# QWERTY6191/projected-lmc

Measured on AMD Instinct MI355X. Metric: MLL+grad iters/sec, n=8192 16-task LMC, higher is better.
Workload: dtype f32; 1 GPU; C3: ProjectedGPModel+ProjectedLMCmll exact training step (PLMC_fast), n=8192 d=8 p=16 q=8 Matern-5/2 fp32; latents sharded q/N per GPU; n_points=8192, n_dim=8, n_tasks=16, n_latents=8, parallelism=latent-shard x1

## Files before the change

projected-lmc_amd/csrc/api_common.hpp:

```cpp
#pragma once
#include <hip/hip_runtime.h>
#include <stdint.h>
#include <stdio.h>
#include <string.h>
#include <type_traits>

#include "gemm_core.hpp"
#include "covariance.hpp"

namespace plmc {

constexpr int MAX_DIM = 32;
constexpr int MAX_COMP = 4;
constexpr int SM_MAX_MIX = 8;
constexpr int SM_MAX_DIM = 8;
constexpr int PER_MAX_DIM = 8;
constexpr int RQ_MAX_DIM = 16;
constexpr int LPER_MAX_DIM = 8;
constexpr int DOT_MAX_DIM = 16;
constexpr int DOT_MAX_POWER = 8;
constexpr int SUM_MAX_DIM = 8;
constexpr int FAM_PUBLIC_BASE = 16;
enum { F_PER = 5, F_RQ = 6, F_LPER = 7 };

// ... 112 lines not shown
  static CovTable add(int kind, int d, int ncomp, const void *ell, const void *oscale) { return {COV_ADD, kind, d, ncomp, ell, nullptr, oscale}; }
  static CovTable sm(int d, int nmix, const void *scales, const void *means, const void *weights) { return {COV_SM, 0, d, nmix, scales, means, weights}; }
  static CovTable per(int d, const void *ell, const void *period, const void *oscale) { return {COV_PER, 0, d, 1, ell, period, oscale}; }
  static CovTable rq(int d, const void *ell, const void *alpha, const void *oscale) { return {COV_RQ, 0, d, 1, ell, alpha, oscale}; }
  static CovTable lper(int d, const void *ell, const void *period, const void *rbf_ell, const void *oscale) {
    return {COV_LPER, 0, d, 1, ell, period, oscale, rbf_ell};
  }
  static CovTable dot(int d, int power, const void *v, const void *c, const void *oscale) { return {COV_DOT, 0, d, power, v, c, oscale}; }
  int power() const { return ncomp; }
  static CovTable sum(int d, int ncomp, const int *fam, const void *table, const void *oscale) {
    CovTable t{COV_SUM, 0, d, ncomp, table, nullptr, oscale};
    if (!fam) t.fams = -3;
    if (!fam || ncomp < 1 || ncomp > MAX_COMP) return t;
    for (int g = 0; g < ncomp; ++g) {
      const int f = fam[g];
      int code;
      if (f >= K_RBF && f <= K_MATERN52) code = f;
      else if (f >= FAM_PUBLIC_BASE && f <= FAM_PUBLIC_BASE + 2) code = F_PER + (f - FAM_PUBLIC_BASE);
      else { t.fams = f == K_SPLINE ? -2 : -1; return t; }
      t.fams |= code << (4 * g);
    }
    return t;
  }
  int fam_of(int g) const { return (fams >> (4 * g)) & 15; }
  CovTable member(const void *ell_, const void *period_, const void *rbf_, const void *alpha_, const void *os_) const {
    const int f = fam_of(0);
    CovTable t = f == F_PER ? per(d, ell_, period_, os_) : f == F_RQ ? rq(d, ell_, alpha_, os_) : f == F_LPER ? lper(d, ell_, period_, rbf_, os_)
                                                                                                          : plain(f, d, ell_, os_);
    t.of_sum = true;
    return t;
  }
  template <typename T> CovTable member_of_latent(int lat) const {
    const T *rec = (const T *)ell + (int64_t)lat * (3 * d + 1);
    return member(rec, rec + d, rec + 2 * d, rec + 3 * d, oscale ? (const T *)oscale + lat : nullptr);
  }
  bool single_member() const { return family == COV_SUM && ncomp == 1; }
  const char *check() const {
    const FamilyTraits &f = FAMILY[family];
    if (family == COV_ADD && (kind < 0 || kind > K_MATERN52)) return "additive kernels take the stationary kinds only (no spline kernel)";
    const char *count = f.max_count && (ncomp < 1 || ncomp > f.max_count) ? f.count_text : nullptr;
    const char *dim = f.max_dim && (d <= 0 || d > f.max_dim) ? f.dim_text : nullptr;
    if (count || dim) return f.count_first ? (count ? count : dim) : (dim ? dim : count);
    if (family == COV_SUM) {
      if (fams == -3 || !ell) return "null pointer";
      if (fams == -2) return "the spline kernel is not a member of a sum (members: the stationary kinds 0..3, PLMC_FAM_PERIODIC, PLMC_FAM_RQ, PLMC_FAM_LPER)";
      if (fams < 0) return "unknown member family code (members: the stationary kinds 0..3, PLMC_FAM_PERIODIC, PLMC_FAM_RQ, PLMC_FAM_LPER; no spectral mixture)";
    }
    return (f.needs_third && !third) || (f.needs_second && !second) ? "null pointer" : nullptr;
  }
  CovFamily route() const { return family == COV_ADD && ncomp == 1 ? COV_PLAIN : family; }
  int partials_rows() const { return FAMILY[family].rows_per_comp ? ncomp : 1; }
  int kernel_kind() const { return family == COV_SUM ? fams : kind; }
  const char *vd_noun() const { return FAMILY[of_sum ? COV_SUM : route()].vd_noun; }
};
#define PLMC_REQUIRE_TABLE(t) \
  do { if (const char *why_ = (t).check()) return plmc::fail(__func__, why_); } while (0)

#define PLMC_LEAD_KIND int kind,
#define PLMC_LEAD_NO_KIND
#define PLMC_UNPACK(...) __VA_ARGS__
#define PLMC_FAMILY_ENTRIES(X, SUF, T)                                                                                                        \
  X(SUF, T, , KIND, (const T *ell, const T *oscale), plmc::CovTable::plain(kind, d, ell, oscale))                                             \
  X(SUF, T, _add, KIND, (int ncomp, const T *ell, const T *oscale), plmc::CovTable::add(kind, d, ncomp, ell, oscale))                         \
  X(SUF, T, _sm, NO_KIND, (int nmix, const T *scales, const T *means, const T *weights), plmc::CovTable::sm(d, nmix, scales, means, weights)) \
  X(SUF, T, _per, NO_KIND, (const T *ell, const T *period, const T *oscale), plmc::CovTable::per(d, ell, period, oscale))                     \
  X(SUF, T, _rq, NO_KIND, (const T *ell, const T *shape, const T *oscale), plmc::CovTable::rq(d, ell, shape, oscale))                         \
  X(SUF, T, _lper, NO_KIND, (const T *ell, const T *period, const T *rbf_ell, const T *oscale),                                               \
    plmc::CovTable::lper(d, ell, period, rbf_ell, oscale))                                                                                    \
  X(SUF, T, _sum, NO_KIND, (int ncomp, const int *fam, const T *table, const T *oscale), plmc::CovTable::sum(d, ncomp, fam, table, oscale))   \
  X(SUF, T, _dot, NO_KIND, (const T *var, const T *offset, int power, const T *oscale), plmc::CovTable::dot(d, power, var, offset, oscale))

struct AssembleJob {
  CovTable table;
  int n;
  const void *X, *noise;
  const void *pnoise = nullptr;
  int64_t stride_pn = 0;
};
#define PLMC_REQUIRE_POINT_NOISE(pnoise, stride_pn, n)                                                                                        \
  do {                                                                                                                                        \
    PLMC_REQUIRE((pnoise) != nullptr, "null pointer");                                                                                        \
    PLMC_REQUIRE((stride_pn) == 0 || (stride_pn) >= (n), "bad sizes (stride_pn is 0, one vector for every latent, or >= n)");                 \
  } while (0)
int assemble_rows(const AssembleJob &job, int elem_bytes, void *A, int64_t lda, int64_t strideA, int q, int ib0, int nrows, void *stream,
                  int ncols = -1, int skip = 0);

hipStream_t side_stream(int which = 0);
hipEvent_t sync_event(int idx);
void bind_sweep_ctx(hipStream_t caller, int e_prev_idx);

inline bool aligned16(const void *p) { return (reinterpret_cast<uintptr_t>(p) & 15) == 0; }

}
```

projected-lmc_amd/csrc/assemble.hip:

```cpp
#include "api_common.hpp"
#include "covariance.hpp"
#include "cov_tables.hpp"
#include "../../include/plmc.h"

namespace plmc {

#define PLMC_ASSEMBLE_BODY(PN)                                                                                                          \
  const int jb = blockIdx.x, ib = ib0 + blockIdx.y, lat = blockIdx.z;                                                                   \
  if (jb < ib || (ib < skip && jb < skip)) return;    \
  extern __shared__ __align__(16) unsigned char smem_raw[];                                                                             \
  T *ui = reinterpret_cast<T *>(smem_raw);                                                                                              \
  const int ldu = d + 1;                                                                                                                \
  T *uj = ui + NB * ldu;                                                                                                                \
  const int tid = threadIdx.x;                                                                                                          \
  const T *el = ell + (int64_t)lat * d;                                                                                                 \
  for (int e = tid; e < NB * d; e += NTHREADS) {                                                                                        \
    int r = e / d, k = e % d;                                                                                                           \
    int gi = ib * NB + r, gj = jb * NB + r;                                                                                             \
    T inv = T(1) / el[k];                                                                                                               \
    ui[r * ldu + k] = gi < n ? X[(int64_t)gi * d + k] * inv : T(0);                                                                     \
    uj[r * ldu + k] = gj < n ? X[(int64_t)gj * d + k] * inv : T(0);                                                                     \
  }                                                                                                                                     \
  __syncthreads();                                                                                                                      \
  const T os = oscale ? oscale[lat] : T(1);                                                                                             \
  const T nz = noise[lat];                                                                                                              \
  T *Al = A + (int64_t)lat * strideA;                                                                                                   \
  const int tx = tid & 15, ty = tid >> 4;                                                                                               \
  _Pragma("unroll 1")                                                                                                                   \
  for (int rr = 0; rr < 8; ++rr) {                                                                                                      \
    const int r = ty + 16 * rr;                                                                                                         \
    const int gi = ib * NB + r;                                                                                                         \
    T pv = T(0);                                                                                                                        \
    if (PN && ib == jb) pv = pnoise[(int64_t)lat * stride_pn + (gi < n ? gi : n - 1)];    \
  _Pragma("unroll")                                                                                                                     \
    for (int h = 0; h < 2; ++h) {                                                                                                       \
      const int c0 = tx * 4 + 64 * h;                                                                                                   \
      T v[4];                                                                                                                           \
  _Pragma("unroll")                                                                                                                     \
      for (int c = 0; c < 4; ++c) {                                                                                                     \
        const int gj = jb * NB + c0 + c;                                                                                                \
        T r2 = T(0), sp = T(1);                                                                                                         \
        for (int k = 0; k < d; ++k) {                                                                                                   \
          T df = ui[r * ldu + k] - uj[(c0 + c) * ldu + k];                                                                              \
          r2 += df * df;                                                                                                                \
          if (kind == K_SPLINE) sp *= spline_factor(ui[r * ldu + k], uj[(c0 + c) * ldu + k]);                                           \
        }                                                                                                                               \
        T val;                                                                                                                          \
        if (gi < n && gj < n) {                                                                                                         \
          val = os * (kind == K_SPLINE ? sp : kern_value<T>(kind, r2));                                                                 \
          if (gi == gj) { val += nz; if (PN) val += pv; }                                                                               \
        } else {                                                                                                                        \
          val = (gi == gj) ? T(1) : T(0);                                         \
        }                                                                                                                               \
        v[c] = val;                                                                                                                     \
      }                                                                                                                                 \
      T *dst = Al + (int64_t)gi * lda + jb * NB + c0;                                  \
      using vec_t = typename Traits<T>::vec_t;                                                                                          \
      constexpr int EPV = Traits<T>::EPV;                                                                                               \
  _Pragma("unroll")                                                                                                                     \
      for (int c = 0; c < 4; c += EPV) {                                                                                                \
        vec_t o;                                                                                                                        \
  _Pragma("unroll")                                                                                                                     \
        for (int e = 0; e < EPV; ++e) o[e] = v[c + e];                                                                                  \
        *reinterpret_cast<vec_t *>(dst + c) = o;                                                                                        \
      }                                                                                                                                 \
    }                                                                                                                                   \
  }
template <typename T>
__global__ __launch_bounds__(NTHREADS) void k_assemble(int kind, const T *__restrict__ X, int n, int d,
                                                        const T *__restrict__ ell, const T *__restrict__ oscale,
                                                        const T *__restrict__ noise, T *__restrict__ A,
                                                        int64_t lda, int64_t strideA, int ib0, int skip) {
  const T *const pnoise = nullptr;
  const int64_t stride_pn = 0;
  PLMC_ASSEMBLE_BODY(false)
}
template <typename T>
__global__ __launch_bounds__(NTHREADS) void k_assemble_pn(int kind, const T *__restrict__ X, int n, int d,
                                                           const T *__restrict__ ell, const T *__restrict__ oscale,
                                                           const T *__restrict__ noise, const T *__restrict__ pnoise, int64_t stride_pn,
                                                           T *__restrict__ A, int64_t lda, int64_t strideA, int ib0, int skip) {
  PLMC_ASSEMBLE_BODY(true)
}

template <typename T, int DCAP, int KIND, class NZ>
__device__ __forceinline__ void assemble_tile(const T *ui, const T *uj, int ldu, T os, NZ nz, T *Al, int64_t lda, int ib,
                                              int jb, int n, bool edge) {
  typedef Pair<T> T2;
  const int tid = threadIdx.x, tx = tid & 31, ty = tid >> 5;
  const int c0 = tx * 4;
  T2 u2[2][DCAP];
#pragma unroll
  for (int pp = 0; pp < 2; ++pp)
#pragma unroll
    for (int k = 0; k < DCAP; ++k) u2[pp][k] = T2{uj[(c0 + 2 * pp) * ldu + k], uj[(c0 + 2 * pp + 1) * ldu + k]};
#pragma unroll 2
  for (int rr = 0; rr < 16; ++rr) {
    const int r = ty + 8 * rr;
    const int gi = ib * NB + r;
    T xi[DCAP];
#pragma unroll
    for (int k = 0; k < DCAP; ++k) xi[k] = ui[r * ldu + k];
    T2 v[2];
#pragma unroll
    for (int pp = 0; pp < 2; ++pp) {
      T2 r2 = {T(0), T(0)};
#pragma unroll
      for (int k = 0; k < DCAP; ++k) {
        const T2 df = xi[k] - u2[pp][k];
        r2 += df * df;
      }
      v[pp] = os * kern_value_pair<T>(KIND, r2);
    }
    T o[4] = {v[0].x, v[0].y, v[1].x, v[1].y};
    if (edge) {
      const auto rn = row_noise<T>(nz, gi, n, ib == jb);
#pragma unroll
      for (int c = 0; c < 4; ++c) {
        const int gj = jb * NB + c0 + c;
        if (gi < n && gj < n) { if (gi == gj) o[c] = add_noise<T>(o[c], rn); }
        else o[c] = (gi == gj) ? T(1) : T(0);
      }
    }
    T *dst = Al + (int64_t)gi * lda + jb * NB + c0;
    using vec_t = typename Traits<T>::vec_t;
    constexpr int EPV = Traits<T>::EPV;
#pragma unroll
    for (int c = 0; c < 4; c += EPV) {
      vec_t w;
#pragma unroll
      for (int e = 0; e < EPV; ++e) w[e] = o[c + e];
      *reinterpret_cast<vec_t *>(dst + c) = w;
    }
  }
}

#define PLMC_ASSEMBLE_SMALL_BODY(PN)                                                                                \
  const int jb = blockIdx.x, ib = ib0 + blockIdx.y, lat = blockIdx.z;                                               \
  if (jb < ib || (ib < skip && jb < skip)) return;                                                                  \
  constexpr int ldu = DCAP + 1;                                                                                     \
  __shared__ T ui[NB * ldu], uj[NB * ldu];                                                                          \
  const int tid = threadIdx.x;                                                                                      \
  const T *el = ell + (int64_t)lat * d;                                                                             \
  for (int e = tid; e < NB * DCAP; e += NTHREADS) {    \
    const int r = e / DCAP, k = e % DCAP;                                                                           \
    const int gi = ib * NB + r, gj = jb * NB + r;                                                                   \
    const T inv = k < d ? T(1) / el[k] : T(0);                                                                      \
    ui[r * ldu + k] = (k < d && gi < n) ? X[(int64_t)gi * d + k] * inv : T(0);                                      \
    uj[r * ldu + k] = (k < d && gj < n) ? X[(int64_t)gj * d + k] * inv : T(0);                                      \
  }                                                                                                                 \
  __syncthreads();                                                                                                  \
  const T os = oscale ? oscale[lat] : T(1);                                                                         \
  const std::conditional_t<PN, PointNoise<T>, T> nz = diag_noise_of<T, PN>(noise, pnoise, stride_pn, lat);          \
  T *Al = A + (int64_t)lat * strideA;                                                                               \
  const bool edge = ib == jb || (jb + 1) * NB > n;                                                                  \
  if (kind == K_RBF) assemble_tile<T, DCAP, K_RBF>(ui, uj, ldu, os, nz, Al, lda, ib, jb, n, edge);                  \
  else if (kind == K_MATERN12) assemble_tile<T, DCAP, K_MATERN12>(ui, uj, ldu, os, nz, Al, lda, ib, jb, n, edge);   \
  else if (kind == K_MATERN32) assemble_tile<T, DCAP, K_MATERN32>(ui, uj, ldu, os, nz, Al, lda, ib, jb, n, edge);   \
  else assemble_tile<T, DCAP, K_MATERN52>(ui, uj, ldu, os, nz, Al, lda, ib, jb, n, edge);
template <typename T, int DCAP>
__global__ __launch_bounds__(NTHREADS) void k_assemble_small(int kind, const T *__restrict__ X, int n, int d,
                                                              const T *__restrict__ ell, const T *__restrict__ oscale,
                                                              const T *__restrict__ noise, T *__restrict__ A,
                                                              int64_t lda, int64_t strideA, int ib0, int skip) {
  const T *const pnoise = nullptr;
  const int64_t stride_pn = 0;
  PLMC_ASSEMBLE_SMALL_BODY(false)
}
template <typename T, int DCAP>
__global__ __launch_bounds__(NTHREADS) void k_assemble_small_pn(int kind, const T *__restrict__ X, int n, int d,
                                                                 const T *__restrict__ ell, const T *__restrict__ oscale,
                                                                 const T *__restrict__ noise, const T *__restrict__ pnoise,
                                                                 int64_t stride_pn, T *__restrict__ A, int64_t lda, int64_t strideA,
                                                                 int ib0, int skip) {
  PLMC_ASSEMBLE_SMALL_BODY(true)
}

template <typename T>
__global__ void k_write_rhs(const T *__restrict__ rhs, int nrhs, int n, T *__restrict__ A, int64_t n_pad,
                            int64_t lda, int64_t strideA, int c0, int64_t naug_pad, int zero_fill) {
  const int lat = blockIdx.y;
  const int64_t idx = (int64_t)blockIdx.x * blockDim.x + threadIdx.x;
  if (idx >= n_pad * naug_pad) return;
  const int64_t i = idx / naug_pad;
  const int c = (int)(idx % naug_pad);
  T *p = A + (int64_t)lat * strideA + i * lda + n_pad + c;
  if (c >= c0 && c < c0 + nrhs) {
    *p = i < n ? rhs[((int64_t)lat * nrhs + (c - c0)) * n + i] : T(0);
  } else if (zero_fill) {
    *p = T(0);
  }
}

constexpr int CROSS_ROWS = 32;
template <typename T, int DCAP>
__global__ __launch_bounds__(NTHREADS) void k_assemble_cross(int kind, const T *__restrict__ X, int n,
                                                              const T *__restrict__ Xs, int ns, int d,
                                                              const T *__restrict__ ell, const T *__restrict__ oscale,
                                                              T *__restrict__ A, int64_t n_rows, int64_t lda,
                                                              int64_t strideA, int64_t col0) {
  __shared__ T xi[CROSS_ROWS][DCAP + 1];
  const int lat = blockIdx.z;
  const int j = blockIdx.x * NTHREADS + threadIdx.x;
  const int64_t i0 = (int64_t)blockIdx.y * CROSS_ROWS;
  const T *el = ell + (int64_t)lat * d;
  for (int e = threadIdx.x; e < CROSS_ROWS * DCAP; e += NTHREADS) {
    const int r = e / DCAP, k = e % DCAP;
    xi[r][k] = (k < d && i0 + r < n) ? X[(i0 + r) * d + k] / el[k] : T(0);
  }
  T xs[DCAP];
#pragma unroll
  for (int k = 0; k < DCAP; ++k) xs[k] = (k < d && j < ns) ? Xs[(int64_t)j * d + k] / el[k] : T(0);
  const T os = oscale ? oscale[lat] : T(1);
  __syncthreads();
  if (j >= ns) return;
  T *out = A + (int64_t)lat * strideA + i0 * lda + col0 + j;
#pragma unroll 4
  for (int r = 0; r < CROSS_ROWS; ++r) {
    if (i0 + r >= n_rows) break;
    T val = T(0);
    if (i0 + r < n) {
      T r2 = T(0), sp = T(1);
#pragma unroll
      for (int k = 0; k < DCAP; ++k) {
        const T df = xi[r][k] - xs[k];
        r2 += df * df;
        if (kind == K_SPLINE && k < d) sp *= spline_factor(xi[r][k], xs[k]);
      }
      val = os * (kind == K_SPLINE ? sp : kern_value<T>(kind, r2));
    }
    out[(int64_t)r * lda] = val;
  }
}

#define PLMC_ASSEMBLE_SMALL_TABLE_BODY(PN)                                                                          \
  const int jb = blockIdx.x, ib = ib0 + blockIdx.y, lat = blockIdx.z;                                               \
  if (jb < ib || (ib < skip && jb < skip)) return;                                                                  \
  constexpr int ldu = DCAP + 1;                                                                                     \
  __shared__ T xi[NB * ldu], xj[NB * ldu], par[P::LDS];                                                             \
  const int tid = threadIdx.x;                                                                                      \
  for (int e = tid; e < NB * DCAP; e += NTHREADS) {    \
    const int r = e / DCAP, k = e % DCAP;                                                                           \
    const int gi = ib * NB + r, gj = jb * NB + r;                                                                   \
    xi[r * ldu + k] = (k < d && gi < n) ? X[(int64_t)gi * d + k] : T(0);                                            \
    xj[r * ldu + k] = (k < d && gj < n) ? X[(int64_t)gj * d + k] : T(0);                                            \
  }                                                                                                                 \
  prm.stage(lat, d, par);                                                                                           \
  __syncthreads();                                                                                                  \
  const std::conditional_t<PN, PointNoise<T>, T> nz = diag_noise_of<T, PN>(noise, pnoise, stride_pn, lat);          \
  T *Al = A + (int64_t)lat * strideA;                                                                               \
  const bool edge = ib == jb || (jb + 1) * NB > n;                                                                  \
  prm.tile(xi, xj, ldu, par, nz, Al, lda, ib, jb, n, edge);
template <typename T, int DCAP, class P>
__global__ __launch_bounds__(NTHREADS) void k_assemble_small_table(const P prm, const T *__restrict__ X, int n, int d,
                                                                    const T *__restrict__ noise, T *__restrict__ A,
                                                                    int64_t lda, int64_t strideA, int ib0, int skip) {
  const T *const pnoise = nullptr;
  const int64_t stride_pn = 0;
  PLMC_ASSEMBLE_SMALL_TABLE_BODY(false)
}
template <typename T, int DCAP, class P>
__global__ __launch_bounds__(NTHREADS) void k_assemble_small_table_pn(const P prm, const T *__restrict__ X, int n, int d,
                                                                       const T *__restrict__ noise, const T *__restrict__ pnoise,
                                                                       int64_t stride_pn, T *__restrict__ A, int64_t lda, int64_t strideA,
                                                                       int ib0, int skip) {
  PLMC_ASSEMBLE_SMALL_TABLE_BODY(true)
}

#define PLMC_ASSEMBLE_ADD_BODY(PN)                                                                                                      \
  const int jb = blockIdx.x, ib = ib0 + blockIdx.y, lat = blockIdx.z;                                                                   \
  if (jb < ib || (ib < skip && jb < skip)) return;                                                                                      \
  extern __shared__ __align__(16) unsigned char smem_raw[];                                                                             \
  T *xi = reinterpret_cast<T *>(smem_raw);                                                                                              \
  const int ldu = d + 1;                                                                                                                \
  T *xj = xi + NB * ldu, *w = xj + NB * ldu, *osl = w + G * d;                                                                          \
  const int tid = threadIdx.x;                                                                                                          \
  for (int e = tid; e < NB * d; e += NTHREADS) {                                                                                        \
    const int r = e / d, k = e % d;                                                                                                     \
    const int gi = ib * NB + r, gj = jb * NB + r;                                                                                       \
    xi[r * ldu + k] = gi < n ? X[(int64_t)gi * d + k] : T(0);                                                                           \
    xj[r * ldu + k] = gj < n ? X[(int64_t)gj * d + k] : T(0);                                                                           \
  }                                                                                                                                     \
  if (tid < G * d) w[tid] = T(1) / ell[(int64_t)lat * G * d + tid];                                                                     \
  if (tid < G) osl[tid] = oscale ? oscale[(int64_t)lat * G + tid] : T(1);                                                               \
  __syncthreads();                                                                                                                      \
  const T nz = noise[lat];                                                                                                              \
  T *Al = A + (int64_t)lat * strideA;                                                                                                   \
  const int tx = tid & 15, ty = tid >> 4;                                                                                               \
  _Pragma("unroll 1")                                                                                                                   \
  for (int rr = 0; rr < 8; ++rr) {                                                                                                      \
    const int r = ty + 16 * rr;                                                                                                         \
    const int gi = ib * NB + r;                                                                                                         \
    T pv = T(0);                                                                                                                        \
    if (PN && ib == jb) pv = pnoise[(int64_t)lat * stride_pn + (gi < n ? gi : n - 1)];    \
  _Pragma("unroll")                                                                                                                     \
    for (int h = 0; h < 2; ++h) {                                                                                                       \
      const int c0 = tx * 4 + 64 * h;                                                                                                   \
      T v[4];                                                                                                                           \
  _Pragma("unroll")                                                                                                                     \
      for (int c = 0; c < 4; ++c) {                                                                                                     \
        const int gj = jb * NB + c0 + c;                                                                                                \
        T val = T(0);                                                                                                                   \
        for (int g = 0; g < G; ++g) {                                                                                                   \
          T r2 = T(0);                                                                                                                  \
          for (int k = 0; k < d; ++k) {                                                                                                 \
            const T sd = (xi[r * ldu + k] - xj[(c0 + c) * ldu + k]) * w[g * d + k];                                                     \
            r2 += sd * sd;                                                                                                              \
          }                                                                                                                             \
          val += osl[g] * kern_value<T>(kind, r2);                                                                                      \
        }                                                                                                                               \
        if (gi < n && gj < n) {                                                                                                         \
          if (gi == gj) { val += nz; if (PN) val += pv; }                                                                               \
        } else {                                                                                                                        \
          val = (gi == gj) ? T(1) : T(0);                                         \
        }                                                                                                                               \
        v[c] = val;                                                                                                                     \
      }                                                                                                                                 \
      T *dst = Al + (int64_t)gi * lda + jb * NB + c0;                                                                                   \
      using vec_t = typename Traits<T>::vec_t;                                                                                          \
      constexpr int EPV = Traits<T>::EPV;                                                                                               \
  _Pragma("unroll")                                                                                                                     \
      for (int c = 0; c < 4; c += EPV) {                                                                                                \
        vec_t o;                                                                                                                        \
  _Pragma("unroll")                                                                                                                     \
        for (int e = 0; e < EPV; ++e) o[e] = v[c + e];                                                                                  \
        *reinterpret_cast<vec_t *>(dst + c) = o;                                                                                        \
      }                                                                                                                                 \
    }                                                                                                                                   \
  }
template <typename T>
__global__ __launch_bounds__(NTHREADS) void k_assemble_add(int kind, const T *__restrict__ X, int n, int d, int G,
                                                            const T *__restrict__ ell, const T *__restrict__ oscale,
                                                            const T *__restrict__ noise, T *__restrict__ A,
                                                            int64_t lda, int64_t strideA, int ib0, int skip) {
  const T *const pnoise = nullptr;
  const int64_t stride_pn = 0;
  PLMC_ASSEMBLE_ADD_BODY(false)
}
template <typename T>
__global__ __launch_bounds__(NTHREADS) void k_assemble_add_pn(int kind, const T *__restrict__ X, int n, int d, int G,
                                                               const T *__restrict__ ell, const T *__restrict__ oscale,
                                                               const T *__restrict__ noise, const T *__restrict__ pnoise, int64_t stride_pn,
                                                               T *__restrict__ A, int64_t lda, int64_t strideA, int ib0, int skip) {
  PLMC_ASSEMBLE_ADD_BODY(true)
}

template <typename T, int DCAP, class P>
__global__ __launch_bounds__(NTHREADS) void k_assemble_cross_table(const P prm, const T *__restrict__ X, int n,
                                                                    const T *__restrict__ Xs, int ns, int d,
                                                                    T *__restrict__ A, int64_t n_rows, int64_t lda,
                                                                    int64_t strideA, int64_t col0) {
  __shared__ T xi[CROSS_ROWS][DCAP + 1];
  __shared__ T par[P::LDS];
  const int lat = blockIdx.z;
  const int j = blockIdx.x * NTHREADS + threadIdx.x;
  const int64_t i0 = (int64_t)blockIdx.y * CROSS_ROWS;
  for (int e = threadIdx.x; e < CROSS_ROWS * DCAP; e += NTHREADS) {
    const int r = e / DCAP, k = e % DCAP;
    xi[r][k] = (k < d && i0 + r < n) ? X[(i0 + r) * d + k] : T(0);
  }
  prm.stage(lat, d, par);
  T xs[DCAP];
#pragma unroll
  for (int k = 0; k < DCAP; ++k) xs[k] = (k < d && j < ns) ? Xs[(int64_t)j * d + k] : T(0);
  __syncthreads();
  if (j >= ns) return;
  T *out = A + (int64_t)lat * strideA + i0 * lda + col0 + j;
#pragma unroll 1
  for (int r = 0; r < CROSS_ROWS; ++r) {
    if (i0 + r >= n_rows) break;
    out[(int64_t)r * lda] = i0 + r < n ? prm.value(xi[r], xs, par) : T(0);
  }
}

template <typename T, int DC, template <typename, int> class P, class... Args>
void launch_small_table(dim3 grid, hipStream_t st, const P<T, DC> &prm, Args... args) {
  hipLaunchKernelGGL((k_assemble_small_table<T, DC, P<T, DC>>), grid, dim3(NTHREADS), 0, st, prm, args...);
}
template <typename T, int DC, template <typename, int> class P, class... Args>
void launch_small_table_pn(dim3 grid, hipStream_t st, const P<T, DC> &prm, Args... args) {
  hipLaunchKernelGGL((k_assemble_small_table_pn<T, DC, P<T, DC>>), grid, dim3(NTHREADS), 0, st, prm, args...);
}
template <typename T, int DC, template <typename, int> class P, class... Args>
void launch_cross_table(dim3 grid, hipStream_t st, const P<T, DC> &prm, Args... args) {
  hipLaunchKernelGGL((k_assemble_cross_table<T, DC, P<T, DC>>), grid, dim3(NTHREADS), 0, st, prm, args...);
}

template <typename T>
int assemble_impl(const CovTable &t, const T *X, int n, const T *noise, const T *pnoise, int64_t stride_pn, T *A, int64_t lda, int64_t strideA,
                  int q, void *stream, int ib0 = 0, int nrows = -1, int ncols = -1, int skip = 0) {
  PLMC_REQUIRE_TABLE(t);
  if (t.single_member()) {
    PLMC_REQUIRE(noise && A && q > 0, "null pointer");
    for (int lat = 0; lat < q; ++lat)
      if (int rc = assemble_impl<T>(t.member_of_latent<T>(lat), X, n, noise + lat, pnoise ? pnoise + (int64_t)lat * stride_pn : nullptr, 0,
                                    A + (int64_t)lat * strideA, lda, strideA, 1, stream, ib0, nrows, ncols, skip))
        return rc;
    return 0;
  }
  const int kind = t.kind, d = t.d;
  const T *ell = (const T *)t.ell, *oscale = (const T *)t.oscale;
  const bool small_only = FAMILY[t.family].max_dim != 0;
  PLMC_REQUIRE(kind >= 0 && kind <= 4, "unknown kernel kind");
  PLMC_REQUIRE(X && ell && noise && A, "null pointer");
  PLMC_REQUIRE(n > 0 && q > 0 && d > 0 && d <= MAX_DIM, small_only ? "need n>0, q>0" : "need n>0, q>0, 0<d<=plmc_max_dim()");
  const int64_t n_pad = plmc_pad(n);
  PLMC_REQUIRE(lda >= n_pad && lda % NB == 0, "lda must be a multiple of NB and >= n_pad");
  PLMC_REQUIRE(strideA >= n_pad * lda || q == 1, "strideA too small");
  const int m = (int)(n_pad / NB);
  if (nrows < 0) nrows = m - ib0;
  if (ncols < 0) ncols = m;
  PLMC_REQUIRE(ib0 >= 0 && nrows >= 0 && ib0 + nrows <= m && ncols <= m && skip >= 0, "row / column range outside the matrix");
  if (nrows == 0 || ncols == 0) return 0;
  const double tiles = (double)nrows * (m - ib0) - (double)nrows * (nrows - 1) / 2.0;
  hipStream_t st = (hipStream_t)stream;
  ProfScope ps(PK_ASSEMBLE, st, 0.0, q * tiles * NB * NB * sizeof(T));
  const dim3 grid(ncols, nrows, q);
  const bool pn = pnoise != nullptr;
  const auto table = [&](const auto &prm) {
    if (pn) launch_small_table_pn(grid, st, prm, X, n, d, noise, pnoise, stride_pn, A, lda, strideA, ib0, skip);
    else launch_small_table(grid, st, prm, X, n, d, noise, A, lda, strideA, ib0, skip);
  };
  const auto small = [&](auto dc) {
    constexpr int DC = decltype(dc)::value;
    if (pn) hipLaunchKernelGGL((k_assemble_small_pn<T, DC>), grid, dim3(NTHREADS), 0, st, kind, X, n, d, ell, oscale, noise, pnoise, stride_pn, A, lda, strideA, ib0, skip);
    else hipLaunchKernelGGL((k_assemble_small<T, DC>), grid, dim3(NTHREADS), 0, st, kind, X, n, d, ell, oscale, noise, A, lda, strideA, ib0, skip);
  };
  switch (t.route()) {
    case COV_PLAIN:
      if (d <= 4 && kind != K_SPLINE)
        small(std::integral_constant<int, 4>());
      else if (d <= 8 && kind != K_SPLINE)
        small(std::integral_constant<int, 8>());
      else if (pn)
        hipLaunchKernelGGL(k_assemble_pn<T>, grid, dim3(NTHREADS), 2 * NB * (d + 1) * sizeof(T), st, kind, X, n, d, ell, oscale, noise, pnoise,
                           stride_pn, A, lda, strideA, ib0, skip);
      else
        hipLaunchKernelGGL(k_assemble<T>, grid, dim3(NTHREADS), 2 * NB * (d + 1) * sizeof(T), st, kind, X, n, d, ell, oscale, noise, A, lda,
                           strideA, ib0, skip);
      break;
    case COV_ADD:
      if (d <= 4) table(device_table<T, COV_ADD, 4>(t));
      else if (d <= 8) table(device_table<T, COV_ADD, 8>(t));
      else if (pn)
        hipLaunchKernelGGL(k_assemble_add_pn<T>, grid, dim3(NTHREADS), (2 * NB * (d + 1) + t.ncomp * d + t.ncomp) * sizeof(T), st, kind, X, n, d,
                           t.ncomp, ell, oscale, noise, pnoise, stride_pn, A, lda, strideA, ib0, skip);
      else
        hipLaunchKernelGGL(k_assemble_add<T>, grid, dim3(NTHREADS), (2 * NB * (d + 1) + t.ncomp * d + t.ncomp) * sizeof(T), st, kind, X, n, d,
                           t.ncomp, ell, oscale, noise, A, lda, strideA, ib0, skip);
      break;
    default:
      with_capacity<0>(t.family, d, [&](auto f, auto dc) { table(device_table<T, decltype(f)::value, decltype(dc)::value>(t)); });
  }
  return launch_status(__func__);
}

template <typename T>
int write_rhs_impl(const T *rhs, int nrhs, int n, T *A, int64_t lda, int64_t strideA, int c0, int clear_cols, int q,
                   void *stream) {
  PLMC_REQUIRE(A && (rhs || nrhs == 0), "null pointer");
  const int64_t n_pad = plmc_pad(n);
  PLMC_REQUIRE(lda > n_pad && lda % NB == 0, "no augmented block (lda must exceed n_pad)");
  PLMC_REQUIRE(c0 >= 0 && nrhs >= 0 && n_pad + c0 + nrhs <= lda, "rhs columns exceed the augmented block");
  PLMC_REQUIRE(clear_cols >= 0 && n_pad + clear_cols <= lda, "clear_cols exceeds the buffer");
  const int64_t ncols = clear_cols > c0 + nrhs ? clear_cols : c0 + nrhs;
  const int zero_fill = clear_cols > 0;
  const int64_t tot = n_pad * ncols;
  ProfScope ps(PK_WRITE_RHS, (hipStream_t)stream, 0.0, q * (double)tot * sizeof(T));
  hipLaunchKernelGGL(k_write_rhs<T>, dim3((unsigned)((tot + 255) / 256), q), dim3(256), 0, (hipStream_t)stream, rhs,
                     nrhs, n, A, n_pad, lda, strideA, c0, ncols, zero_fill);
  return launch_status(__func__);
}

template <typename T>
int assemble_cross_impl(const CovTable &t, const T *X, int n, const T *Xs, int ns, T *Out, int64_t ldo, int64_t strideO, int64_t col0,
                        int64_t n_rows, int q, void *stream) {
  PLMC_REQUIRE_TABLE(t);
  if (t.single_member()) {
    PLMC_REQUIRE(Out && q > 0, "null pointer");
    for (int lat = 0; lat < q; ++lat)
      if (int rc = assemble_cross_impl<T>(t.member_of_latent<T>(lat), X, n, Xs, ns, Out + (int64_t)lat * strideO, ldo, strideO, col0, n_rows, 1, stream))
        return rc;
    return 0;
  }
  const int kind = t.kind, d = t.d;
  const T *ell = (const T *)t.ell, *oscale = (const T *)t.oscale;
  PLMC_REQUIRE(kind >= 0 && kind <= 4, "unknown kernel kind");
  PLMC_REQUIRE(X && Xs && ell && Out, "null pointer");
  PLMC_REQUIRE(n > 0 && ns > 0 && q > 0 && d > 0 && d <= MAX_DIM, "bad sizes");
  PLMC_REQUIRE(n_rows >= n && col0 >= 0 && col0 + ns <= ldo, "cross block exceeds the output buffer");
  hipStream_t st = (hipStream_t)stream;
  ProfScope ps(PK_CROSS, st, 0.0, q * (double)n_rows * ns * sizeof(T));
  const dim3 grid((ns + NTHREADS - 1) / NTHREADS, (unsigned)((n_rows + CROSS_ROWS - 1) / CROSS_ROWS), q);
  const auto table = [&](const auto &prm) { launch_cross_table(grid, st, prm, X, n, Xs, ns, d, Out, n_rows, ldo, strideO, col0); };
  const auto plain = [&](auto dc) {
    hipLaunchKernelGGL((k_assemble_cross<T, decltype(dc)::value>), grid, dim3(NTHREADS), 0, st, kind, X, n, Xs, ns, d, ell, oscale, Out, n_rows, ldo,
                       strideO, col0);
  };
  switch (t.route()) {
    case COV_PLAIN:
      if (d <= 4) plain(std::integral_constant<int, 4>());
      else if (d <= 8) plain(std::integral_constant<int, 8>());
      else if (d <= 16) plain(std::integral_constant<int, 16>());
      else plain(std::integral_constant<int, 32>());
      break;
    case COV_ADD:
      if (d <= 4) table(device_table<T, COV_ADD, 4>(t));
      else if (d <= 8) table(device_table<T, COV_ADD, 8>(t));
      else if (d <= 16) table(device_table<T, COV_ADD, 16>(t));
      else table(device_table<T, COV_ADD, 32>(t));
      break;
    default:
      with_capacity<0>(t.family, d, [&](auto f, auto dc) { table(device_table<T, decltype(f)::value, decltype(dc)::value>(t)); });
  }
  return launch_status(__func__);
}

int assemble_rows(const AssembleJob &job, int elem_bytes, void *A, int64_t lda, int64_t strideA, int q, int ib0, int nrows, void *stream,
                  int ncols, int skip) {
  if (elem_bytes == 4)
    return assemble_impl<float>(job.table, (const float *)job.X, job.n, (const float *)job.noise, (const float *)job.pnoise, job.stride_pn, (float *)A,
                                lda, strideA, q, stream, ib0, nrows, ncols, skip);
  return assemble_impl<double>(job.table, (const double *)job.X, job.n, (const double *)job.noise, (const double *)job.pnoise, job.stride_pn,
                               (double *)A, lda, strideA, q, stream, ib0, nrows, ncols, skip);
}
}

extern "C" {
int plmc_write_rhs_f32(const float *rhs, int nrhs, int n, float *A, int64_t lda, int64_t strideA, int c0,
                       int clear_cols, int q, void *stream) {
  return plmc::write_rhs_impl<float>(rhs, nrhs, n, A, lda, strideA, c0, clear_cols, q, stream);
}
// ... 33 lines not shown
```

projected-lmc_amd/csrc/potrf.hip:

```cpp
#include <stdlib.h>
#include "api_common.hpp"
#include "covariance.hpp"
#include "diag_block.hpp"
#include "bf3_engine.hpp"
#include "chain_engine.hpp"
#include "vd_layout.hpp"
#include "../../include/plmc.h"

namespace plmc {

template <typename T> constexpr int CHAIN_BURST = sizeof(T) == 8 ? 4 : 8;

template <typename T> struct ColMap {
  int u0, nU, Taug, w0, nW;
  int64_t n_pad;
  T *W;
  int64_t ldw, strideW;
};

template <typename T, int NT, bool BURSTED = false>
__global__ __launch_bounds__(NTHREADS, TILE_MIN_WAVES<T>) void k_panel(T *A, int64_t lda, int64_t strideA, int r, ColMap<T> cm,
                                                     const T *__restrict__ Vd, int64_t strideV) {
  __builtin_amdgcn_s_setprio(3);
  __shared__ __align__(16) T smem[tile_smem_elems<T>()];
// ... 864 lines not shown
    }
  }
  void raw_planes0(hipStream_t s, const ColMap<T> &cm) {
    if constexpr (bf3) {
      const int nt = cm.nU + cm.Taug + cm.nW;
      if (nt > 0)
        hipLaunchKernelGGL((k_raw_planes<S>), dim3(nt, G0(1), q), dim3(NTHREADS), 0, s, (const float *)A, lda, strideA, 0, cm, Praw, pl_lat, wcol0,
                           (const float *)scl, sc_lat);
    }
  }

  void near(int gi, hipStream_t s) {
    const int g1 = G0(gi + 1), g2 = G0(gi + 2), g3 = G0(gi + 3);
    update(g2, g3 - g2, pair_lo(gi), g1 - 1, cm_buf(g2, m - g2, Taug, 0, g1), s, PK_TRAIL, 0, 0, false, 0, true);
  }
  void far(int gi, hipStream_t s) {
    if (!(gi & 1)) return;
    const int g1 = G0(gi + 1), g3 = G0(gi + 3);
    update(g3, m - g3, pair_lo(gi), g1 - 1, cm_buf(g3, m - g3, Taug, 0, g1), s, PK_TRAIL);
  }

  bool bind_streams() {
    if (!kn.serial) bind_sweep_ctx(st, 8);
    C = kn.serial ? nullptr : side_stream();
    H = kn.serial ? nullptr : (kn.bulk_streams == 1 ? st : side_stream(1));
    hipEvent_t *const ev[] = {&e_entry, &e_v, &e_gh, &e_p, &e_hd, &e_tail, &e_doneC, &e_doneH, &e_prev};
    bool la = C && H && ng > 2;
    for (int i = 0; i < 9; ++i) la = (*ev[i] = sync_event(i)) && la;
    e_sc = sync_event(12);
    return la;
  }

  int inputs(const AssembleJob *job) {
    if (job) {
      const int rc = assemble_rows(*job, (int)sizeof(T), A, lda, strideA, q, 0, m, st);
      if (rc != 0) return rc;
    }
    scan(st, 0, n_pad, 0, SCAN_PARTS);
    split_scales(st);
    return 0;
  }

  int one_stream(const AssembleJob *job) {
    const int rc = inputs(job);
    if (rc != 0) return rc;
    raw_planes0(st, cm_buf(G0(1), m - G0(1), Taug, 0, 0));
    for (int gi = 0; gi < ng; ++gi) {
      const int g0 = G0(gi), g1 = G0(gi + 1), g2 = G0(gi + 2);
      chain(gi, st);
      vtrans(gi, st);
      wtri_planes(gi, st);
      if (bf3) {
        gpanel(g0, g1 - g0, cm_buf(g1, g2 - g1, 0, 0, 0), gi & 1, st, 1);
        gpanel(g0, g1 - g0, cm_buf(g2, m - g2, Taug, 0, g0), gi & 1, st, 0);
        if (pair) {
          update(g1, g2 - g1, g0, g1 - 1, cm_buf(g2, m - g2, Taug, 0, g1), st, PK_TRAIL_HEAD, 0, 0, false, g2);
          near(gi, st);
          far(gi, st);
        } else {
          update(g1, m - g1, g0, g1 - 1, cm_buf(g1, m - g1, Taug, 0, g1), st, PK_TRAIL, g2, g2, false, g2);
        }
        update(g1, g2 - g1, g0, g1 - 1, cm_buf(g1, g2 - g1, 0, 0, 0), st, PK_TRAIL_HEAD, 0, 0, true);
      } else {
        gpanel(g0, g1 - g0, cm_buf(g1, m - g1, Taug, 0, g0), gi & 1, st, 0);
        update(g1, m - g1, g0, g1 - 1, cm_buf(g1, m - g1, Taug, 0, g1), st, PK_TRAIL);
      }
    }
    return finish(st);
  }

  int lookahead(const AssembleJob *job) {
    const bool fused = job && e_sc;
    if (fused) {
      const int rc = assemble_rows(*job, (int)sizeof(T), A, lda, strideA, q, 0, G0(1), st, G0(1));
      if (rc != 0) return rc;
      scan(st, 0, (int64_t)G0(1) * NB, 0, SCAN_PARTS / 2);
    } else {
      const int rc = inputs(job);
      if (rc != 0) return rc;
    }
    (void)hipEventRecord(e_entry, st);
    (void)hipStreamWaitEvent(C, e_entry, 0);
    (void)hipStreamWaitEvent(H, e_entry, 0);
    if (fused) {
      const int rc = assemble_rows(*job, (int)sizeof(T), A, lda, strideA, q, 0, m, H, -1, G0(1));
      if (rc != 0) return rc;
      scan(H, (int64_t)G0(1) * NB, n_pad, SCAN_PARTS / 2, SCAN_PARTS / 2);
      split_scales(H);
      (void)hipEventRecord(e_sc, H);
    }
    raw_planes0(H, cm_buf(G0(1), m - G0(1), Taug, 0, 0));
    (void)hipEventRecord(e_hd, H);
    for (int gi = 0; gi < ng; ++gi) {
      const int g0 = G0(gi), g1 = G0(gi + 1), g2 = G0(gi + 2), G = g1 - g0;
      chain(gi, C);
      if (fused && gi == 0) (void)hipStreamWaitEvent(C, e_sc, 0);
      vtrans(gi, C);
      (void)hipEventRecord(e_v, C);
      if (gi > 0 || bf3) (void)hipStreamWaitEvent(C, e_hd, 0);
      gpanel(g0, G, cm_buf(g1, g2 - g1, 0, 0, 0), gi & 1, C, 1);
      (void)hipEventRecord(e_gh, C);
      if (gi > 0) (void)hipStreamWaitEvent(C, e_tail, 0);
      update(g1, g2 - g1, g0, g1 - 1, cm_buf(g1, g2 - g1, 0, 0, 0), C, PK_TRAIL_HEAD, 0, 0, true);

      (void)hipStreamWaitEvent(H, e_v, 0);
      wtri_planes(gi, H);
      gpanel(g0, G, cm_buf(g2, m - g2, Taug, 0, g0), gi & 1, H, 0);
      (void)hipEventRecord(e_p, H);
      (void)hipStreamWaitEvent(H, e_gh, 0);
      if (gi > 0) (void)hipStreamWaitEvent(H, e_tail, 0);
      update(g1, g2 - g1, g0, g1 - 1, cm_buf(g2, m - g2, Taug, 0, g1), H, PK_TRAIL_HEAD, 0, 0, false, g2);
      (void)hipEventRecord(e_hd, H);

      (void)hipStreamWaitEvent(st, e_p, 0);
      (void)hipStreamWaitEvent(st, e_gh, 0);
      if (pair) {
        near(gi, st);
        (void)hipEventRecord(e_tail, st);
        far(gi, st);
      } else {
        update(g2, m - g2, g0, g1 - 1, cm_buf(g2, m - g2, Taug, 0, g1), st, PK_TRAIL);
        (void)hipEventRecord(e_tail, st);
      }
    }
    const int rc_fin = finish(C);
    (void)hipEventRecord(e_doneC, C);
    (void)hipEventRecord(e_doneH, H);
    (void)hipStreamWaitEvent(st, e_doneC, 0);
    (void)hipStreamWaitEvent(st, e_doneH, 0);
    (void)hipEventRecord(e_prev, st);
    return rc_fin;
  }
};

template <typename T, class S>
int potrf_impl(T *A, int64_t n_pad, int64_t lda, int naug, int64_t strideA, T *Vd, double *logdet, int *info,
               int with_inverse_arg, int q, const float *eig_lo, void *stream, const AssembleJob *job = nullptr) {
  PLMC_REQUIRE((with_inverse_arg & 2) == 0, "with_inverse bit 1 (K^-1 accumulated in the sweep) is gone: use plmc_kinv_grad_* behind the sweep");
  const bool with_inverse = (with_inverse_arg & 1) != 0;
  const bool keep = !std::is_void<S>::value && (with_inverse_arg & 4) != 0 && with_inverse;
  PLMC_REQUIRE(A && Vd && logdet && info, "null pointer");
  PLMC_REQUIRE(n_pad > 0 && n_pad % NB == 0 && lda % NB == 0 && lda >= n_pad, "n_pad/lda must be multiples of NB");
  const int64_t naug_pad = plmc_pad(naug);
  PLMC_REQUIRE(naug >= 0 && n_pad + naug_pad + (with_inverse ? n_pad : 0) <= lda,
               "lda too small for naug (+ the n_pad columns of the inverse factor)");
  PLMC_REQUIRE(q > 0 && aligned16(A) && aligned16(Vd), "bad q or unaligned buffer");
  const Knobs &kn = knobs();
  const int grp = (!keep && kn.grp > 0 && kn.grp < GMAX) ? kn.grp : GMAX;
  const unsigned bulk_lds = (unsigned)(kn.bulk_lds >= 0 ? kn.bulk_lds : (q == 1 ? 20000 : (q == 2 ? 16000 : 0)));
  Sweep<T, S> sw(A, n_pad, lda, naug, n_pad + naug_pad, strideA, Vd, q, with_inverse, keep, grp, bulk_lds, (hipStream_t)stream);
  sw.eig_lo = eig_lo;
  sw.logdet = logdet;
  sw.info = info;
  const double npd = (double)n_pad;
  ProfScope whole(PK_SWEEP, sw.st, q * (with_inverse ? 2.0 : 1.0) * npd * npd * npd / 3.0, 0.0);
  sw.clear();
  return sw.bind_streams() ? sw.lookahead(job) : sw.one_stream(job);
}

bool vd_w_planes(const float *Vd, int64_t n_pad, int64_t lda, const unsigned short **wk, int64_t *wk_lat_stride, const float **w_scale,
                 int64_t *w_scale_lat_stride) {
  const VdLayout L(n_pad, lda, 4, false);
  if (L.wk < 0) return false;
  *wk = L.at<const unsigned short>(Vd, L.wk);
  *wk_lat_stride = L.stride_u16();
  *w_scale = L.at<const float>(Vd, L.scl) + SC_SW;
  *w_scale_lat_stride = L.stride_f32();
  return true;
}

template <typename T>
int potrs_aug_at(T *A, int64_t n_pad, int64_t lda, int naug, int64_t wcol0, int64_t strideA, T *Vd, int q, void *stream) {
  PLMC_REQUIRE(A && Vd, "null pointer");
  PLMC_REQUIRE(n_pad > 0 && n_pad % NB == 0 && lda % NB == 0 && wcol0 % NB == 0, "n_pad / lda / wcol0 must be multiples of NB");
  const int64_t naug_pad = plmc_pad(naug);
  PLMC_REQUIRE(naug > 0 && q > 0 && n_pad + naug_pad <= wcol0 && wcol0 + n_pad <= lda, "augmented columns must fit between the square part and the W columns");
  PLMC_REQUIRE(aligned16(A) && aligned16(Vd), "unaligned buffer");
  Sweep<T, void> sw(A, n_pad, lda, naug, wcol0, strideA, Vd, q, true, false, GMAX, 0u, (hipStream_t)stream);
  const ColMap<T> cm{0, 0, sw.Taug, 0, 0, n_pad, (T *)nullptr, lda, strideA};
  for (int gi = 0; gi < sw.ng; ++gi) {
    const int g0 = sw.G0(gi), g1 = sw.G0(gi + 1), G = g1 - g0;
    hipLaunchKernelGGL((k_vtrans<T, void>), dim3(G * (G + 1) / 2, q), dim3(NTHREADS), 0, sw.st, (const T *)(sw.WA + (int64_t)g0 * NB * lda + (int64_t)g0 * NB),
// ... 187 lines not shown
```

Before: 61.51 iters/sec.

## Assemble diagonal tiles first and split remaining assembly across streams

Adds a diagonal-only assembly mode, so the scale scan can start after only the diagonal tiles of the trailing rows are built instead of waiting for full assembly. The remaining row ranges are then assembled on the main stream and the helper stream, overlapping with the first chain and panel steps. An extra event wait is added on the chain stream when fused. This reorders cross-stream dependencies, which risks races if any consumer reads rows before they are written, and adds more launches.

```diff
diff --git a/projected-lmc_amd/csrc/api_common.hpp b/projected-lmc_amd/csrc/api_common.hpp
--- a/projected-lmc_amd/csrc/api_common.hpp
+++ b/projected-lmc_amd/csrc/api_common.hpp
@@ -218,6 +218,7 @@
     PLMC_REQUIRE((pnoise) != nullptr, "null pointer");                                                                                        \
     PLMC_REQUIRE((stride_pn) == 0 || (stride_pn) >= (n), "bad sizes (stride_pn is 0, one vector for every latent, or >= n)");                 \
   } while (0)
+constexpr int ASSEMBLE_DIAG = -2;
 int assemble_rows(const AssembleJob &job, int elem_bytes, void *A, int64_t lda, int64_t strideA, int q, int ib0, int nrows, void *stream,
                   int ncols = -1, int skip = 0);
 
diff --git a/projected-lmc_amd/csrc/assemble.hip b/projected-lmc_amd/csrc/assemble.hip
--- a/projected-lmc_amd/csrc/assemble.hip
+++ b/projected-lmc_amd/csrc/assemble.hip
@@ -6,7 +6,7 @@
 namespace plmc {
 
 #define PLMC_ASSEMBLE_BODY(PN)                                                                                                          \
-  const int jb = blockIdx.x, ib = ib0 + blockIdx.y, lat = blockIdx.z;                                                                   \
+  const int ib = ib0 + blockIdx.y, jb = diag ? ib : (int)blockIdx.x, lat = blockIdx.z;                                                  \
   if (jb < ib || (ib < skip && jb < skip)) return;    \
   extern __shared__ __align__(16) unsigned char smem_raw[];                                                                             \
   T *ui = reinterpret_cast<T *>(smem_raw);                                                                                              \
@@ -70,7 +70,7 @@
 __global__ __launch_bounds__(NTHREADS) void k_assemble(int kind, const T *__restrict__ X, int n, int d,
                                                         const T *__restrict__ ell, const T *__restrict__ oscale,
                                                         const T *__restrict__ noise, T *__restrict__ A,
-                                                        int64_t lda, int64_t strideA, int ib0, int skip) {
+                                                        int64_t lda, int64_t strideA, int ib0, int skip, int diag) {
   const T *const pnoise = nullptr;
   const int64_t stride_pn = 0;
   PLMC_ASSEMBLE_BODY(false)
@@ -79,7 +79,7 @@
 __global__ __launch_bounds__(NTHREADS) void k_assemble_pn(int kind, const T *__restrict__ X, int n, int d,
                                                            const T *__restrict__ ell, const T *__restrict__ oscale,
                                                            const T *__restrict__ noise, const T *__restrict__ pnoise, int64_t stride_pn,
-                                                           T *__restrict__ A, int64_t lda, int64_t strideA, int ib0, int skip) {
+                                                           T *__restrict__ A, int64_t lda, int64_t strideA, int ib0, int skip, int diag) {
   PLMC_ASSEMBLE_BODY(true)
 }
 
@@ -136,7 +136,7 @@
 }
 
 #define PLMC_ASSEMBLE_SMALL_BODY(PN)                                                                                \
-  const int jb = blockIdx.x, ib = ib0 + blockIdx.y, lat = blockIdx.z;                                               \
+  const int ib = ib0 + blockIdx.y, jb = diag ? ib : (int)blockIdx.x, lat = blockIdx.z;                              \
   if (jb < ib || (ib < skip && jb < skip)) return;                                                                  \
   constexpr int ldu = DCAP + 1;                                                                                     \
   __shared__ T ui[NB * ldu], uj[NB * ldu];                                                                          \
@@ -162,7 +162,7 @@
 __global__ __launch_bounds__(NTHREADS) void k_assemble_small(int kind, const T *__restrict__ X, int n, int d,
                                                               const T *__restrict__ ell, const T *__restrict__ oscale,
                                                               const T *__restrict__ noise, T *__restrict__ A,
-                                                              int64_t lda, int64_t strideA, int ib0, int skip) {
+                                                              int64_t lda, int64_t strideA, int ib0, int skip, int diag) {
   const T *const pnoise = nullptr;
   const int64_t stride_pn = 0;
   PLMC_ASSEMBLE_SMALL_BODY(false)
@@ -172,7 +172,7 @@
                                                                  const T *__restrict__ ell, const T *__restrict__ oscale,
                                                                  const T *__restrict__ noise, const T *__restrict__ pnoise,
                                                                  int64_t stride_pn, T *__restrict__ A, int64_t lda, int64_t strideA,
-                                                                 int ib0, int skip) {
+                                                                 int ib0, int skip, int diag) {
   PLMC_ASSEMBLE_SMALL_BODY(true)
 }
 
@@ -234,7 +234,7 @@
 }
 
 #define PLMC_ASSEMBLE_SMALL_TABLE_BODY(PN)                                                                          \
-  const int jb = blockIdx.x, ib = ib0 + blockIdx.y, lat = blockIdx.z;                                               \
+  const int ib = ib0 + blockIdx.y, jb = diag ? ib : (int)blockIdx.x, lat = blockIdx.z;                              \
   if (jb < ib || (ib < skip && jb < skip)) return;                                                                  \
   constexpr int ldu = DCAP + 1;                                                                                     \
   __shared__ T xi[NB * ldu], xj[NB * ldu], par[P::LDS];                                                             \
@@ -254,7 +254,7 @@
 template <typename T, int DCAP, class P>
 __global__ __launch_bounds__(NTHREADS) void k_assemble_small_table(const P prm, const T *__restrict__ X, int n, int d,
                                                                     const T *__restrict__ noise, T *__restrict__ A,
-                                                                    int64_t lda, int64_t strideA, int ib0, int skip) {
+                                                                    int64_t lda, int64_t strideA, int ib0, int skip, int diag) {
   const T *const pnoise = nullptr;
   const int64_t stride_pn = 0;
   PLMC_ASSEMBLE_SMALL_TABLE_BODY(false)
@@ -263,12 +263,12 @@
 __global__ __launch_bounds__(NTHREADS) void k_assemble_small_table_pn(const P prm, const T *__restrict__ X, int n, int d,
                                                                        const T *__restrict__ noise, const T *__restrict__ pnoise,
                                                                        int64_t stride_pn, T *__restrict__ A, int64_t lda, int64_t strideA,
-                                                                       int ib0, int skip) {
+                                                                       int ib0, int skip, int diag) {
   PLMC_ASSEMBLE_SMALL_TABLE_BODY(true)
 }
 
 #define PLMC_ASSEMBLE_ADD_BODY(PN)                                                                                                      \
-  const int jb = blockIdx.x, ib = ib0 + blockIdx.y, lat = blockIdx.z;                                                                   \
+  const int ib = ib0 + blockIdx.y, jb = diag ? ib : (int)blockIdx.x, lat = blockIdx.z;                                                  \
   if (jb < ib || (ib < skip && jb < skip)) return;                                                                                      \
   extern __shared__ __align__(16) unsigned char smem_raw[];                                                                             \
   T *xi = reinterpret_cast<T *>(smem_raw);                                                                                              \
@@ -332,7 +332,7 @@
 __global__ __launch_bounds__(NTHREADS) void k_assemble_add(int kind, const T *__restrict__ X, int n, int d, int G,
                                                             const T *__restrict__ ell, const T *__restrict__ oscale,
                                                             const T *__restrict__ noise, T *__restrict__ A,
-                                                            int64_t lda, int64_t strideA, int ib0, int skip) {
+                                                            int64_t lda, int64_t strideA, int ib0, int skip, int diag) {
   const T *const pnoise = nullptr;
   const int64_t stride_pn = 0;
   PLMC_ASSEMBLE_ADD_BODY(false)
@@ -341,7 +341,7 @@
 __global__ __launch_bounds__(NTHREADS) void k_assemble_add_pn(int kind, const T *__restrict__ X, int n, int d, int G,
                                                                const T *__restrict__ ell, const T *__restrict__ oscale,
                                                                const T *__restrict__ noise, const T *__restrict__ pnoise, int64_t stride_pn,
-                                                               T *__restrict__ A, int64_t lda, int64_t strideA, int ib0, int skip) {
+                                                               T *__restrict__ A, int64_t lda, int64_t strideA, int ib0, int skip, int diag) {
   PLMC_ASSEMBLE_ADD_BODY(true)
 }
 
@@ -409,22 +409,24 @@
   PLMC_REQUIRE(strideA >= n_pad * lda || q == 1, "strideA too small");
   const int m = (int)(n_pad / NB);
   if (nrows < 0) nrows = m - ib0;
+  const int diag = ncols == ASSEMBLE_DIAG;
+  if (diag) ncols = 1;
   if (ncols < 0) ncols = m;
   PLMC_REQUIRE(ib0 >= 0 && nrows >= 0 && ib0 + nrows <= m && ncols <= m && skip >= 0, "row / column range outside the matrix");
   if (nrows == 0 || ncols == 0) return 0;
-  const double tiles = (double)nrows * (m - ib0) - (double)nrows * (nrows - 1) / 2.0;
+  const double tiles = diag ? (double)nrows : (double)nrows * (m - ib0) - (double)nrows * (nrows - 1) / 2.0;
   hipStream_t st = (hipStream_t)stream;
   ProfScope ps(PK_ASSEMBLE, st, 0.0, q * tiles * NB * NB * sizeof(T));
   const dim3 grid(ncols, nrows, q);
   const bool pn = pnoise != nullptr;
   const auto table = [&](const auto &prm) {
-    if (pn) launch_small_table_pn(grid, st, prm, X, n, d, noise, pnoise, stride_pn, A, lda, strideA, ib0, skip);
-    else launch_small_table(grid, st, prm, X, n, d, noise, A, lda, strideA, ib0, skip);
+    if (pn) launch_small_table_pn(grid, st, prm, X, n, d, noise, pnoise, stride_pn, A, lda, strideA, ib0, skip, diag);
+    else launch_small_table(grid, st, prm, X, n, d, noise, A, lda, strideA, ib0, skip, diag);
   };
   const auto small = [&](auto dc) {
     constexpr int DC = decltype(dc)::value;
-    if (pn) hipLaunchKernelGGL((k_assemble_small_pn<T, DC>), grid, dim3(NTHREADS), 0, st, kind, X, n, d, ell, oscale, noise, pnoise, stride_pn, A, lda, strideA, ib0, skip);
-    else hipLaunchKernelGGL((k_assemble_small<T, DC>), grid, dim3(NTHREADS), 0, st, kind, X, n, d, ell, oscale, noise, A, lda, strideA, ib0, skip);
+    if (pn) hipLaunchKernelGGL((k_assemble_small_pn<T, DC>), grid, dim3(NTHREADS), 0, st, kind, X, n, d, ell, oscale, noise, pnoise, stride_pn, A, lda, strideA, ib0, skip, diag);
+    else hipLaunchKernelGGL((k_assemble_small<T, DC>), grid, dim3(NTHREADS), 0, st, kind, X, n, d, ell, oscale, noise, A, lda, strideA, ib0, skip, diag);
   };
   switch (t.route()) {
     case COV_PLAIN:
@@ -434,20 +436,20 @@
         small(std::integral_constant<int, 8>());
       else if (pn)
         hipLaunchKernelGGL(k_assemble_pn<T>, grid, dim3(NTHREADS), 2 * NB * (d + 1) * sizeof(T), st, kind, X, n, d, ell, oscale, noise, pnoise,
-                           stride_pn, A, lda, strideA, ib0, skip);
+                           stride_pn, A, lda, strideA, ib0, skip, diag);
       else
         hipLaunchKernelGGL(k_assemble<T>, grid, dim3(NTHREADS), 2 * NB * (d + 1) * sizeof(T), st, kind, X, n, d, ell, oscale, noise, A, lda,
-                           strideA, ib0, skip);
+                           strideA, ib0, skip, diag);
       break;
     case COV_ADD:
       if (d <= 4) table(device_table<T, COV_ADD, 4>(t));
       else if (d <= 8) table(device_table<T, COV_ADD, 8>(t));
       else if (pn)
         hipLaunchKernelGGL(k_assemble_add_pn<T>, grid, dim3(NTHREADS), (2 * NB * (d + 1) + t.ncomp * d + t.ncomp) * sizeof(T), st, kind, X, n, d,
-                           t.ncomp, ell, oscale, noise, pnoise, stride_pn, A, lda, strideA, ib0, skip);
+                           t.ncomp, ell, oscale, noise, pnoise, stride_pn, A, lda, strideA, ib0, skip, diag);
       else
         hipLaunchKernelGGL(k_assemble_add<T>, grid, dim3(NTHREADS), (2 * NB * (d + 1) + t.ncomp * d + t.ncomp) * sizeof(T), st, kind, X, n, d,
-                           t.ncomp, ell, oscale, noise, A, lda, strideA, ib0, skip);
+                           t.ncomp, ell, oscale, noise, A, lda, strideA, ib0, skip, diag);
       break;
     default:
       with_capacity<0>(t.family, d, [&](auto f, auto dc) { table(device_table<T, decltype(f)::value, decltype(dc)::value>(t)); });
diff --git a/projected-lmc_amd/csrc/potrf.hip b/projected-lmc_amd/csrc/potrf.hip
--- a/projected-lmc_amd/csrc/potrf.hip
+++ b/projected-lmc_amd/csrc/potrf.hip
@@ -970,14 +970,24 @@
     (void)hipEventRecord(e_entry, st);
     (void)hipStreamWaitEvent(C, e_entry, 0);
     (void)hipStreamWaitEvent(H, e_entry, 0);
+    const auto rows = [&](hipStream_t s, int ib0, int ib1) {
+      return assemble_rows(*job, (int)sizeof(T), A, lda, strideA, q, ib0, ib1 - ib0, s, -1, G0(1));
+    };
     if (fused) {
-      const int rc = assemble_rows(*job, (int)sizeof(T), A, lda, strideA, q, 0, m, H, -1, G0(1));
+      int rc = assemble_rows(*job, (int)sizeof(T), A, lda, strideA, q, G0(1), m - G0(1), H, ASSEMBLE_DIAG);
       if (rc != 0) return rc;
       scan(H, (int64_t)G0(1) * NB, n_pad, SCAN_PARTS / 2, SCAN_PARTS / 2);
       split_scales(H);
       (void)hipEventRecord(e_sc, H);
+      (void)hipStreamWaitEvent(st, e_sc, 0);
+      if ((rc = rows(st, G0(2), m)) != 0) return rc;
+      if ((rc = rows(H, 0, G0(1))) != 0) return rc;
     }
     raw_planes0(H, cm_buf(G0(1), m - G0(1), Taug, 0, 0));
+    if (fused) {
+      const int rc = rows(H, G0(1), G0(2));
+      if (rc != 0) return rc;
+    }
     (void)hipEventRecord(e_hd, H);
     for (int gi = 0; gi < ng; ++gi) {
       const int g0 = G0(gi), g1 = G0(gi + 1), g2 = G0(gi + 2), G = g1 - g0;
@@ -985,7 +995,7 @@
       if (fused && gi == 0) (void)hipStreamWaitEvent(C, e_sc, 0);
       vtrans(gi, C);
       (void)hipEventRecord(e_v, C);
-      if (gi > 0 || bf3) (void)hipStreamWaitEvent(C, e_hd, 0);
+      if (gi > 0 || bf3 || fused) (void)hipStreamWaitEvent(C, e_hd, 0);
       gpanel(g0, G, cm_buf(g1, g2 - g1, 0, 0, 0), gi & 1, C, 1);
       (void)hipEventRecord(e_gh, C);
       if (gi > 0) (void)hipStreamWaitEvent(C, e_tail, 0);
```

Result: no change. 61.52 iters/sec, median of 2 (+0.0%).
